# mahbhlddnhakkh/yuv-manipulations-2

Hardware: AMD Instinct MI355X
Metric: megapixels/sec DCT compress+decompress, 4K IYUV; achieved HBM GB/s vs peak (higher is better)
Workload: dtype u8/int16 (fp32 transform)

## Files before the change

### yuv-manipulations-2_amd/csrc/fdct_bfly.h

```cpp
#pragma once

#if defined(__HIPCC__)
#define MYYUV_BF_HD __host__ __device__ __forceinline__
#else
#include <math.h>
#define MYYUV_BF_HD static inline
#endif

#ifndef MYYUV_BFLY_MUTANT
#define MYYUV_BFLY_MUTANT 0
#endif
#if MYYUV_BFLY_MUTANT && defined(__HIPCC__)
#error "MYYUV_BFLY_MUTANT is for the host check only"
#endif
#if MYYUV_BFLY_MUTANT == 1
#define MYYUV_BF_FMA(a, b, c) ((a) * (b) + (c))
#else
#define MYYUV_BF_FMA(a, b, c) fmaf(a, b, c)
#endif

namespace myyuv_bfly {

#if MYYUV_BFLY_MUTANT == 2
constexpr float kC0 = 0.3535533845424652f, kC4 = kC0;
#else
constexpr float kC0 = 0.3535533845424652f, kC4 = 0.3535534143447876f;
#endif
constexpr float kA2 = 0.4619397521018982f, kB2 = 0.19134166836738586f;
constexpr float kA6 = 0.4619397521018982f, kB6 = 0.19134169816970825f;
constexpr float kO1[4] = {0.49039262533187866f, 0.41573476791381836f, 0.27778512239456177f, 0.09754513204097748f};
constexpr float kO3[4] = {0.41573482751846313f, -0.0975450873374939f, -0.49039262533187866f, -0.277785062789917f};
constexpr float kO5[4] = {0.2777852416038513f, -0.49039262533187866f, 0.09754514694213867f, 0.41573476791381836f};
constexpr float kO7[4] = {0.09754543751478195f, -0.2777852416038513f, 0.4157347083091736f, -0.49039262533187866f};
constexpr float kBflyK = 7.946e-7f;

MYYUV_BF_HD float odd4(const float (&o)[4], float d0, float d1, float d2, float d3) {
  return MYYUV_BF_FMA(o[3], d3, MYYUV_BF_FMA(o[2], d2, MYYUV_BF_FMA(o[1], d1, o[0] * d0)));
}

MYYUV_BF_HD void bfly_cols(const float (&p)[8], float (&t)[8]) {
  const float s0 = p[0] + p[7], s1 = p[1] + p[6], s2 = p[2] + p[5], s3 = p[3] + p[4];
  const float d0 = p[0] - p[7], d1 = p[1] - p[6], d2 = p[2] - p[5], d3 = p[3] - p[4];
  const float ss0 = s0 + s3, ss1 = s1 + s2, ds0 = s0 - s3, ds1 = s1 - s2;
  t[0] = kC0 * ((ss0 + ss1) - 1024.0f);
  t[4] = kC4 * (ss0 - ss1);
  t[2] = MYYUV_BF_FMA(kA2, ds0, kB2 * ds1);
  t[6] = MYYUV_BF_FMA(kB6, ds0, -kA6 * ds1);
  t[1] = odd4(kO1, d0, d1, d2, d3);
  t[3] = odd4(kO3, d0, d1, d2, d3);
  t[5] = odd4(kO5, d0, d1, d2, d3);
  t[7] = odd4(kO7, d0, d1, d2, d3);
}

MYYUV_BF_HD void bfly_rows(const float (&x)[8], float (&y)[8]) {
  const float s0 = x[0] + x[7], s1 = x[1] + x[6], s2 = x[2] + x[5], s3 = x[3] + x[4];
  const float d0 = x[0] - x[7], d1 = x[1] - x[6], d2 = x[2] - x[5], d3 = x[3] - x[4];
  const float ss0 = s0 + s3, ss1 = s1 + s2, ds0 = s0 - s3, ds1 = s1 - s2;
  y[0] = kC0 * (ss0 + ss1);
  y[4] = kC4 * (ss0 - ss1);
  y[2] = MYYUV_BF_FMA(kA2, ds0, kB2 * ds1);
  y[6] = MYYUV_BF_FMA(kB6, ds0, -kA6 * ds1);
  y[1] = odd4(kO1, d0, d1, d2, d3);
  y[3] = odd4(kO3, d0, d1, d2, d3);
  y[5] = odd4(kO5, d0, d1, d2, d3);
  y[7] = odd4(kO7, d0, d1, d2, d3);
}

MYYUV_BF_HD void bfly_row_bounds(const float* r, float* kb) {
  for (int i = 0; i < 8; i++) {
    double m = 0.0;
    for (int v = 0; v < 8; v++) m = r[i * 8 + v] > m ? r[i * 8 + v] : m;
    kb[i] = (float)((double)kBflyK * m * (1.0 + 0x1p-20) * (1.0 + 0x1p-22));
  }
}

#if !defined(__HIPCC__)
struct BflyDetail {
  int row, col;
  float dec;
  float a;
  float t[64];
};
static inline int bfly_block(const unsigned char* px, const float* R, const float* kb, short* out,
                             BflyDetail* d = nullptr) {
  unsigned a = 0;
  for (int i = 0; i < 64; i++) a += px[i] > 128 ? px[i] - 128u : 128u - px[i];
  const float af = (float)a;
  float T[8][8];
  for (int k = 0; k < 8; k++) {
    float p[8], t[8];
    for (int m = 0; m < 8; m++) p[m] = (float)px[m * 8 + k];
    bfly_cols(p, t);
    for (int i = 0; i < 8; i++) T[i][k] = t[i];
  }
  int ok = 1;
  for (int i = 0; i < 8; i++) {
    float y[8];
    bfly_rows(T[i], y);
    float em = 0.0f;
    int vm = 0;
    for (int v = 0; v < 8; v++) {
      const float t = y[v] * R[i * 8 + v];
      const float uu = t + 0x1.8p23f;
      const float e = t - (uu - 0x1.8p23f);
      if (fabsf(e) > em) vm = v;
      em = fmaxf(em, fabsf(e));
      out[i * 8 + v] = (short)(int)(uu - 0x1.8p23f);
      if (d) d->t[i * 8 + v] = t;
    }
    const float dec = fmaf(af, kb[i], em);
    if (dec >= 0.5f) ok = 0;
    if (d && (i == 0 || dec > d->dec)) {
      d->row = i;
      d->col = vm;
      d->dec = dec;
    }
  }
  if (d) d->a = af;
  return ok;
}
#endif

}
```

### yuv-manipulations-2_amd/csrc/k1_store.hpp

```cpp
#pragma once
#include "codec_common.hpp"
#include "xform_common.hpp"

namespace myyuv_gpu {
namespace xf {

typedef unsigned short k1_us2 __attribute__((ext_vector_type(2)));

__device__ __forceinline__ void store_block_rows(const uint32_t (&c)[16], uint32_t q, uint32_t lane, bool live,
                                                 uint32_t g, uint4* dlo, uint4* dhi, uint8_t* __restrict__ rmask,
                                                 uint32_t* __restrict__ binfo, const uint4* zq,
                                                 uint4* __restrict__ sink) {
  uint4 lo, hi;
  uint32_t rm;
  pack_quads(c, q, lo, hi, rm);
  const uint4 z0 = zq[0], z1 = zq[1];
  const uint32_t wv[8] = {lo.x, lo.y, lo.z, lo.w, hi.x, hi.y, hi.z, hi.w};
  const uint32_t zv[8] = {z0.x, z0.y, z0.z, z0.w, z1.x, z1.y, z1.z, z1.w};
  k1_us2 cnt = {0, 0}, mx = {0, 0};
#pragma unroll
  for (int i = 0; i < 8; i++) {
    uint32_t fu, m16;
    asm("v_pk_min_u16 %0, %1, %2" : "=v"(fu) : "v"(wv[i]), "s"(0x00010001u));
    cnt += __builtin_bit_cast(k1_us2, fu);
    asm("v_pk_mul_lo_u16 %0, %1, %2" : "=v"(m16) : "v"(fu), "v"(zv[i]));
    mx = __builtin_elementwise_max(mx, __builtin_bit_cast(k1_us2, m16));
  }
  uint32_t nnz = (uint32_t)cnt.x + (uint32_t)cnt.y;
  uint32_t msz = mx.x > mx.y ? (uint32_t)mx.x : (uint32_t)mx.y;
#pragma unroll
  for (int d = 1; d < 4; d <<= 1) {
    const uint32_t o = d == 1 ? quad_xor1(nnz | (msz << 16)) : quad_xor2(nnz | (msz << 16));
    nnz += o & 0xFFFFu;
    msz = max(msz, o >> 16);
  }
  const bool nzl = (rm >> (2 * q)) & 1u, nzh = (rm >> (2 * q + 1)) & 1u;
  *(live ? rmask + g : reinterpret_cast<uint8_t*>(sink + 128) + lane) = (uint8_t)rm;
  const uint32_t dc = quad_lane0(lo.x);
  *(live ? binfo + g : reinterpret_cast<uint32_t*>(sink + 132) + lane) = binfo_word(rm, msz, class_of(nnz, msz), dc);
  *(nzl ? dlo : sink + lane) = lo;
  *(nzh ? dhi : sink + 64 + lane) = hi;
}

#ifndef MYYUV_K1_BUF
#define MYYUV_K1_BUF 1
#endif
typedef unsigned int k1_v4u __attribute__((ext_vector_type(4)));
constexpr uint32_t kOob = 0xFFFFFFFFu;

struct K1Rsrc {
  __amdgpu_buffer_rsrc_t coef, rmask, binfo;
};
__device__ __forceinline__ K1Rsrc k1_rsrc(uint4* coef, uint8_t* rmask, uint32_t* binfo, const FrameGeom& G) {
  const uint32_t nblk = G.cum[3] * G.nframes;
  K1Rsrc r;
  r.coef = __builtin_amdgcn_make_buffer_rsrc(coef, 0, (int)(((nblk + 63u) / 64u) * (kCoefQuadsPerWave * 16u)),
                                             0x00020000);
  r.rmask = __builtin_amdgcn_make_buffer_rsrc(rmask, 0, (int)nblk, 0x00020000);
  r.binfo = __builtin_amdgcn_make_buffer_rsrc(binfo, 0, (int)(nblk * 4u), 0x00020000);
  return r;
}

__device__ __forceinline__ void store_block_rows_buf(const uint32_t (&c)[16], uint32_t q, bool live, uint32_t g,
                                                     const K1Rsrc& R, const uint4* zq) {
  uint4 lo, hi;
  uint32_t rm;
  pack_quads(c, q, lo, hi, rm);
  const uint4 z0 = zq[0], z1 = zq[1];
  const uint32_t wv[8] = {lo.x, lo.y, lo.z, lo.w, hi.x, hi.y, hi.z, hi.w};
  const uint32_t zv[8] = {z0.x, z0.y, z0.z, z0.w, z1.x, z1.y, z1.z, z1.w};
  k1_us2 cnt = {0, 0}, mx = {0, 0};
#pragma unroll
  for (int i = 0; i < 8; i++) {
    uint32_t fu, m16;
    asm("v_pk_min_u16 %0, %1, %2" : "=v"(fu) : "v"(wv[i]), "s"(0x00010001u));
    cnt += __builtin_bit_cast(k1_us2, fu);
    asm("v_pk_mul_lo_u16 %0, %1, %2" : "=v"(m16) : "v"(fu), "v"(zv[i]));
    mx = __builtin_elementwise_max(mx, __builtin_bit_cast(k1_us2, m16));
  }
  uint32_t nnz = (uint32_t)cnt.x + (uint32_t)cnt.y;
  uint32_t msz = mx.x > mx.y ? (uint32_t)mx.x : (uint32_t)mx.y;
#pragma unroll
  for (int d = 1; d < 4; d <<= 1) {
    const uint32_t o = d == 1 ? quad_xor1(nnz | (msz << 16)) : quad_xor2(nnz | (msz << 16));
    nnz += o & 0xFFFFu;
    msz = max(msz, o >> 16);
  }
  const bool nzl = (rm >> (2 * q)) & 1u, nzh = (rm >> (2 * q + 1)) & 1u;
  const uint32_t dc = quad_lane0(lo.x);
  __builtin_amdgcn_raw_buffer_store_b8((uint8_t)rm, R.rmask, live ? g : kOob, 0, 0);
  __builtin_amdgcn_raw_buffer_store_b32(binfo_word(rm, msz, class_of(nnz, msz), dc), R.binfo, live ? 4u * g : kOob,
                                        0, 0);
  const uint32_t qo = coef_quad(g, 2 * q) * 16u;
  __builtin_amdgcn_raw_buffer_store_b128(k1_v4u{lo.x, lo.y, lo.z, lo.w}, R.coef, live && nzl ? qo : kOob, 0, 0);
  __builtin_amdgcn_raw_buffer_store_b128(k1_v4u{hi.x, hi.y, hi.z, hi.w}, R.coef, live && nzh ? qo + 1024u : kOob, 0,
                                         0);
}

__device__ __forceinline__ void stage_zz(uint4* szz) {
  if (threadIdx.x < 32) reinterpret_cast<uint32_t*>(szz)[threadIdx.x] = kZzPairs.v[threadIdx.x];
}

}
}
```

### yuv-manipulations-2_amd/csrc/k_huff_decode.hip

```cpp
#include "codec_common.hpp"
#include "coef_xform.h"
#include "downscale.h"
#include "huff_common.hpp"
#include "idct_scaled.h"
#include "k1_store.hpp"
#include "k_metric.hpp"
#include "k_stream.hpp"
#include "requant.h"
#include "xform_common.hpp"

namespace myyuv_gpu {

namespace {

constexpr uint32_t kStageQuads = 320;
constexpr uint32_t kZeroBit = kStageQuads * 128u;
constexpr uint32_t kGposQuads = 8 * 64 * 4 / 16;

#ifndef MYYUV_K5_GROUP
#define MYYUV_K5_GROUP 2
#endif
#ifndef MYYUV_K5_FORMS
#define MYYUV_K5_FORMS 1
#endif
// ... 1259 lines not shown
        const uint32_t w = v < 2 ? w0 : w1;
        z[u * N + v] = (int16_t)((v & 1) ? w >> 16 : w & 0xFFFFu);
        q[u * N + v] = sqs[8 * u + v];
      }
    }
    uint8_t px[N * N];
    myyuv_scaled::idct_scaled_block<N>(z, q, px);
    if (live) {
#pragma unroll
      for (int i = 0; i < N; i++) {
        uint8_t* o = img + myyuv_downscale::lane_pixel(kDen, r, lane, (uint32_t)i);
        if constexpr (N == 1) {
          o[0] = px[0];
        } else if constexpr (N == 2) {
          *reinterpret_cast<uint16_t*>(o) = (uint16_t)(px[2 * i] | (px[2 * i + 1] << 8));
        } else {
          *reinterpret_cast<uint32_t*>(o) = (uint32_t)px[4 * i] | ((uint32_t)px[4 * i + 1] << 8) |
                                            ((uint32_t)px[4 * i + 2] << 16) | ((uint32_t)px[4 * i + 3] << 24);
        }
      }
    }
  }
  xf::wave_sync();

  const uint32_t q = lane & 3u, b = lane >> 2;
  float* tb = reinterpret_cast<float*>(stq) + b * xf::kTile;
  const xf::K1Rsrc rs = xf::k1_rsrc(coef, rmask, binfo, Gd);
  const uint32_t g0 = blockIdx.y * Gd.cum[3] + (p == 0 ? Gd.cum[0] : (p == 1 ? Gd.cum[1] : Gd.cum[2]));
#pragma unroll 1
  for (uint32_t u0 = 0; u0 < W.nout; u0 += kXfUnit) {
    const uint32_t slot = u0 + b;
    const bool lv = slot < W.nout;
    const uint32_t g = g0 + myyuv_downscale::out_block(W, slot);
    xf::fdct_core(img + 64u * slot, tb, q, sqr, p, [&](const uint32_t (&c)[16], bool keep) {
      xf::store_block_rows_buf(c, q, lv && keep, g, rs, szz + 2 * q);
    });
    xf::wave_sync();
  }
}
#define MYYUV_DOWNSCALE_INST(N)                                                                                   \
  template __global__ void k_downscale<N>(const uint8_t*, const uint32_t*, uint32_t, const StreamDesc*,           \
                                          const uint32_t*, const uint32_t*, FrameGeom, FrameGeom,                 \
                                          myyuv_downscale::Map, const DownscaleTables*, uint4*, uint8_t*,         \
                                          uint32_t*, unsigned long long*);
MYYUV_DOWNSCALE_INST(1)
MYYUV_DOWNSCALE_INST(2)
MYYUV_DOWNSCALE_INST(4)
#undef MYYUV_DOWNSCALE_INST

__global__ __launch_bounds__(64, MYYUV_K5_WAVES) void k_requant(const uint8_t* __restrict__ in,
                                               const uint32_t* __restrict__ in_size,
                                               uint32_t cap,
                                               const StreamDesc* __restrict__ desc,
                                               const uint32_t* __restrict__ local_off,
                                               const uint32_t* __restrict__ tile_pre,
                                               FrameGeom G, uint32_t tiles_p0,
                                               uint32_t tiles_p1, const RequantTables* __restrict__ rt,
                                               uint4* __restrict__ coef,
                                               uint8_t* __restrict__ rmask,
                                               uint32_t* __restrict__ binfo,
                                               unsigned long long* __restrict__ err) {
  __shared__ uint4 stq[kStageQuads + 1 + kGposQuads];
  __shared__ float sqs[64], sqd[64];
  const uint32_t lane = threadIdx.x;
  if (lane == 0) stq[kStageQuads] = make_uint4(0u, 0u, 0u, 0u);
  {
    const uint32_t t = blockIdx.x;
    const int p = t >= tiles_p0 ? (t >= tiles_p0 + tiles_p1 ? 2 : 1) : 0;
// ... 305 lines not shown
```

### yuv-manipulations-2_amd/csrc/k_huff_encode.hip

```cpp
#include "codec_common.hpp"
#ifdef MYYUV_STAMPS
namespace myyuv_gpu {
extern __device__ uint32_t g_k2_fstamps[8192 * 8];
}
#define R8_STAMP_DECL unsigned long long _r8prev = 0;
#define R8_STAMP(k)                                                                   \
  do {                                                                                \
    __builtin_amdgcn_sched_barrier(0);                                                \
    unsigned long long _t = __builtin_amdgcn_s_memtime();                             \
    __builtin_amdgcn_sched_barrier(0);                                                \
    if ((threadIdx.x & 63) == 0 && (k) > 0 && blockIdx.x * (blockDim.x >> 6) + (threadIdx.x >> 6) < 8192) \
      g_k2_fstamps[(blockIdx.x * (blockDim.x >> 6) + (threadIdx.x >> 6)) * 8 + (k)] = (uint32_t)(_t - _r8prev); \
    _r8prev = _t;                                                                     \
  } while (0)
#endif
#include "huff_common.hpp"
#include "huff_r16.hpp"
#include "xform_common.hpp"

namespace myyuv_gpu {

#ifdef MYYUV_STAMPS
__device__ unsigned long long g_k2_stamps[40];
__device__ uint32_t g_k2_fstamps[8192 * 8];
// ... 1127 lines not shown
                                                             const QTables* __restrict__ qt,
                                                             uint4* __restrict__ coef,
                                                             uint8_t* __restrict__ rmask,
                                                             uint32_t* __restrict__ stage,
                                                             uint32_t* __restrict__ tinfo,
                                                             uint8_t* __restrict__ sizes,
                                                             uint32_t* __restrict__ srcoff,
                                                             uint32_t* __restrict__ work,
                                                             uint32_t* __restrict__ work_count) {
  using namespace xf;
  __shared__ uint4 s_img[8 * kK2Group];
  __shared__ float s_tile[kTileWaves][kXfUnit * kTile];
  __shared__ float s_q[kSqWords];
  __shared__ uint8_t s_rmk[kK2Group];
  static_assert(sizeof(TileScratch) <= sizeof(s_tile), "K2 scratch over the transpose tiles");
  const uint32_t tid = threadIdx.x, wave = tid >> 6, lane = tid & 63;
  const uint32_t q = lane & 3u, b = lane >> 2;
  const uint32_t T = blockIdx.y * G.tcum[3] + blockIdx.x;
  uint32_t f, t, g0, nloc;
  int p;
  tile_geometry(G, T, f, t, p, g0, nloc);
  TileRows rows;
  load_tile_rows(frame, G, T, wave, b, q, rows);
  stage_tables<kSqWords>(qt->q[0], s_q);
  float* tb = s_tile[wave] + b * kTile;
  uint8_t* img = reinterpret_cast<uint8_t*>(tb);
#pragma unroll
  for (int i = 0; i < 4; i++) {
    const uint32_t lb = (4 * wave + i) * kXfUnit + b;
    if ((4 * wave + i) * kXfUnit >= nloc) break;
    *reinterpret_cast<uint2*>(img + 16u * q) = make_uint2(rows.px[i].x, rows.px[i].y);
    *reinterpret_cast<uint2*>(img + 16u * q + 8u) = make_uint2(rows.px[i].z, rows.px[i].w);
    wave_sync();
    fdct_core(img, tb, q, s_q, p, [&](const uint32_t (&c)[16], bool) {
      uint4 lo, hi;
      uint32_t rm;
      pack_quads(c, q, lo, hi, rm);
      if (lb < nloc) {
        s_img[(2 * q) * kK2Group + lb] = lo;
        s_img[(2 * q + 1) * kK2Group + lb] = hi;
        if (q == 0) s_rmk[lb] = (uint8_t)rm;
      }
    });
    wave_sync();
  }
  __syncthreads();
  TileScratch& sc = *reinterpret_cast<TileScratch*>(&s_tile[0][0]);
  const LdsCoef src{s_img, s_rmk, coef, rmask, f * G.cum[3] + g0};
  encode_tile(src, sc, T, nloc, stage, tinfo, sizes, srcoff, work, work_count);
}

__global__ __launch_bounds__(kWideLanes) void k_huff_encode_wide(const uint4* __restrict__ coef,
                                                        const uint8_t* __restrict__ rmask,
                                                        const uint4* __restrict__ zq, FrameGeom G,
                                                        uint32_t* __restrict__ oslots,
                                                        uint8_t* __restrict__ sizes,
                                                        uint32_t* __restrict__ tinfo,
                                                        const uint32_t* __restrict__ work,
                                                        const uint32_t* __restrict__ work_count,
                                                        const uint32_t* __restrict__ work2,
                                                        const uint32_t* __restrict__ work2_count,
                                                        uint32_t gate, uint32_t limit) {
  constexpr int CAP = 64;
  __shared__ uint32_t lds[Layout<CAP>::kWords * kWideLanes];
  const OvfList L = overflow_list(work, work_count, work2, work2_count, gate);
  const uint32_t cnt = L.n;
  if (cnt <= limit) return;
  for (uint32_t base = blockIdx.x * kWideLanes; base < cnt; base += gridDim.x * kWideLanes) {
    const uint32_t i = base + threadIdx.x;
    const bool live = i < cnt;
    const uint32_t g = live ? L.ids[i] : 0;
    CoefRegs R;
    R.load(coef, zq, g, live ? rmask[g] : 0u);
// ... 77 lines not shown
```

### yuv-manipulations-2_amd/csrc/k_transform.hip

```cpp
#include <stddef.h>

#include "bmp_fdct.h"
#include "codec_common.hpp"
#include "color_px.hpp"
#include "k1_store.hpp"
#include "k_metric.hpp"
#include "xform_common.hpp"

#ifndef MYYUV_K1_OCC
#define MYYUV_K1_OCC 8
#endif
#define MYYUV_K1_ATTR __attribute__((amdgpu_waves_per_eu(MYYUV_K1_OCC, MYYUV_K1_OCC)))

namespace myyuv_gpu {

using namespace xf;



__global__ __launch_bounds__(256) MYYUV_K1_ATTR void k_fdct_quant(const uint8_t* __restrict__ frame, FrameGeom G,
                                                   const QTables* __restrict__ qt,
                                                   uint4* __restrict__ coef, uint8_t* __restrict__ rmask,
                                                   uint32_t* __restrict__ binfo, uint4* __restrict__ sink,
                                                   uint32_t* __restrict__ k2ctl, uint32_t* __restrict__ fix,
// ... 2 lines not shown
  __shared__ float tile[4][kXfUnit * kTile];
  __shared__ float sqr[kSqWords];
  __shared__ uint4 szz[8];
  static_assert(offsetof(QTables, r) == sizeof(float) * kSqR && offsetof(QTables, kb) == sizeof(float) * kSqKb,
                "layout");
  stage_zz(szz);
  stage_tables<kSqWords>(qt->q[0], sqr);
  if (kSinkSlots > 1) sink += (size_t)((blockIdx.x * 4u + (threadIdx.x >> 6)) % kSinkSlots) * kSinkQuads;
  const uint32_t lane = threadIdx.x & 63u;
  const uint32_t q = lane & 3u, b = lane >> 2;
  float* tb = tile[threadIdx.x >> 6] + b * kTile;
  uint8_t* img = reinterpret_cast<uint8_t*>(tb);
#if MYYUV_K1_BUF
  const K1Rsrc rs = k1_rsrc(coef, rmask, binfo, G);
#endif
  const uint32_t nall = G.ucum[3] * G.nframes, stride = unit_stride();
  uint32_t ua = first_unit();
  uint4 nx = ua < nall ? load_rows(frame, G, ua, b, q) : make_uint4(0, 0, 0, 0);
  sink[lane] = make_uint4(0, 0, 0, 0);
  sink[64 + lane] = make_uint4(0, 0, 0, 0);
  reinterpret_cast<uint8_t*>(sink + 128)[lane] = 0;

  for (; ua < nall; ua += stride) {
    const uint32_t f = div_magic(ua, G.umag);
    const Unit U = unit_of(G, ua - f * G.ucum[3]);
    const uint32_t local = U.local0 + b;
    const bool live = local < U.nb;
    const uint32_t g = f * G.cum[3] + U.cum + local;
    *reinterpret_cast<uint2*>(img + 16u * q) = make_uint2(nx.x, nx.y);
    *reinterpret_cast<uint2*>(img + 16u * q + 8u) = make_uint2(nx.z, nx.w);
    nx = load_rows(frame, G, ua + stride < nall ? ua + stride : ua, b, q);
    wave_sync();

    auto store = [&](const uint32_t (&c)[16], bool keep) {
      const bool lv = live && keep;
#if MYYUV_K1_BUF
      store_block_rows_buf(c, q, lv, g, rs, szz + 2 * q);
#else
      uint4* dlo = lv ? coef + coef_quad(g, 2 * q) : sink + lane;
      uint4* dhi = lv ? coef + coef_quad(g, 2 * q + 1) : sink + 64 + lane;
      store_block_rows(c, q, lane, lv, g, dlo, dhi, rmask, binfo, szz + 2 * q, sink);
#endif
    };
    uint32_t xr[4];
    fdct_load(img, q, xr);
    const uint64_t bad = fdct_fast<true>(xr, tb, q, sqr, U.p, store);
    if (bad != 0) {
      const bool mine = ((bad >> lane) & 1u) && q == 0 && live;
      const uint64_t m = __ballot(mine);
      const uint32_t c = ua % kFixLists;
      uint32_t base = 0;
      if (lane == 0 && m != 0) base = atomicAdd(fix_count(fix, par, c), (uint32_t)__popcll(m));
      base = __builtin_amdgcn_readfirstlane(base);
      const uint32_t idx = base + __builtin_amdgcn_mbcnt_hi((uint32_t)(m >> 32), __builtin_amdgcn_mbcnt_lo((uint32_t)m, 0u));
      if (mine && idx < fix_list_cap(nall)) fix_list(fix, G, c)[idx] = ua * kXfUnit + b;
    }
  }
}

__global__ __launch_bounds__(64 * kFixWaves) void k_fdct_fix(const uint8_t* __restrict__ frame, FrameGeom G,
                                                  const QTables* __restrict__ qt, uint4* __restrict__ coef,
                                                  uint8_t* __restrict__ rmask, uint32_t* __restrict__ binfo,
                                                  uint4* __restrict__ sink,
                                                  uint32_t* __restrict__ fix, uint32_t par) {
  __shared__ float tile[kFixWaves][kXfUnit * kTile];
  __shared__ float sqr[2 * 3 * 64];
  __shared__ uint4 szz[8];
  __shared__ uint32_t s_any;
  if (blockIdx.x == 0 && threadIdx.x < kFixLists) *fix_count(fix, par ^ 1u, threadIdx.x) = 0u;
  if (threadIdx.x == 0) s_any = 0u;
  __syncthreads();
  const uint32_t gw = blockIdx.x * kFixWaves + (threadIdx.x >> 6), nw = gridDim.x * kFixWaves;
  const uint32_t c = gw % kFixLists;
  const uint32_t n = __builtin_amdgcn_readfirstlane(*fix_count(fix, par, c));
  if ((threadIdx.x & 63u) == 0 && gw / kFixLists * kXfUnit < n) s_any = 1u;
  __syncthreads();
  if (s_any == 0u) return;
  stage_zz(szz);
#pragma unroll
  for (uint32_t i = threadIdx.x; i < 2u * 3u * 64u; i += 64u * kFixWaves) sqr[i] = qt->q[0][i];
  __syncthreads();
  const uint32_t lane = threadIdx.x & 63u;
  const uint32_t q = lane & 3u, b = lane >> 2;
  float* tb = tile[threadIdx.x >> 6] + b * kTile;
  uint8_t* img = reinterpret_cast<uint8_t*>(tb);
  const uint32_t* list = fix_list(fix, G, c);
#if MYYUV_K1_BUF
  const K1Rsrc rs = k1_rsrc(coef, rmask, binfo, G);
#endif
  for (uint32_t i = gw / kFixLists * kXfUnit; i < n; i += nw / kFixLists * kXfUnit) {
    const bool real = i + b < n;
    const uint32_t ent = list[real ? i + b : i];
    const uint32_t ua = ent / kXfUnit, bb = ent % kXfUnit;
    const uint32_t f = div_magic(ua, G.umag);
    const Unit U = unit_of(G, ua - f * G.ucum[3]);
    const uint32_t g = f * G.cum[3] + U.cum + U.local0 + bb;
    const uint4 r = load_rows(frame, G, ua, bb, q);
    wave_sync();
    *reinterpret_cast<uint2*>(img + 16u * q) = make_uint2(r.x, r.y);
    *reinterpret_cast<uint2*>(img + 16u * q + 8u) = make_uint2(r.z, r.w);
    wave_sync();
    uint32_t xr[4];
    fdct_load(img, q, xr);
#if MYYUV_K1_BUF
    fdct_exact(xr, tb, q, sqr, U.p, [&](const uint32_t (&cc)[16]) { store_block_rows_buf(cc, q, real, g, rs, szz + 2 * q); });
#else
    uint4* dlo = real ? coef + coef_quad(g, 2 * q) : sink + lane;
    uint4* dhi = real ? coef + coef_quad(g, 2 * q + 1) : sink + 64 + lane;
    fdct_exact(xr, tb, q, sqr, U.p,
               [&](const uint32_t (&cc)[16]) {
                 store_block_rows(cc, q, lane, real, g, dlo, dhi, rmask, binfo, szz + 2 * q, sink);
               });
#endif
  }
}

template <class Out>
__device__ __forceinline__ void dequant_idct_units(const uint4* __restrict__ coef,
                                                   const uint8_t* __restrict__ rmask,
                                                   const uint4* __restrict__ zq, const FrameGeom& G,
                                                   float (*tile)[kXfUnit * kTile], const float* sq,
                                                   uint4* __restrict__ sink, Out& out) {
  const uint32_t lane = threadIdx.x & 63u;
  const uint32_t q = lane & 3u, b = lane >> 2;
  float* tb = tile[threadIdx.x >> 6] + b * kTile;
  uint32_t* tw = reinterpret_cast<uint32_t*>(tb);
  const uint32_t nall = G.ucum[3] * G.nframes, stride = unit_stride();
  uint32_t ua = first_unit();
  uint4 na = make_uint4(0, 0, 0, 0), nc = na;
  uint32_t un = ua + stride < nall ? ua + stride : ua, nm = 0;
  if (ua < nall) {
    const uint32_t g0 = unit_block(G, ua, b);
    load_quads(coef, zq, g0, q, rmask[g0], na, nc);
    nm = rmask[unit_block(G, un, b)];
  }
  sink[lane] = make_uint4(0, 0, 0, 0);
  sink[64 + lane] = make_uint4(0, 0, 0, 0);

  for (; ua < nall; ua += stride) {
    const uint32_t f = div_magic(ua, G.umag);
    const Unit U = unit_of(G, ua - f * G.ucum[3]);
    const uint32_t local = U.local0 + b;
    *reinterpret_cast<uint4*>(tw + 8 * q) = na;
    *reinterpret_cast<uint4*>(tw + 8 * q + 4) = nc;
// ... 184 lines not shown
    for (uint32_t t0 = 0; t0 < bf::kTileRows; t0 += kDepth) {
      uint32_t w[kDepth][2][BPP];
#pragma unroll
      for (uint32_t i = 0; i < kDepth; i++)
#pragma unroll
        for (uint32_t dr = 0; dr < 2; dr++) px::load4<BPP>(fr + (int64_t)(2 * (t0 + i) + dr) * step, 0, w[i][dr]);
#pragma unroll
      for (uint32_t i = 0; i < kDepth; i++) {
        const uint32_t ty = t0 + i;
        uint32_t Y[2] = {0, 0}, cb[2] = {0, 0}, cr[2] = {0, 0};
        px::tile_row<BPP>(w[i][0], M.orient == 1, Y[0], cb, cr);
        px::tile_row<BPP>(w[i][1], M.orient == 1, Y[1], cb, cr);
        *reinterpret_cast<uint32_t*>(img + bf::luma_byte(S, lane, ty, 0)) = Y[0];
        *reinterpret_cast<uint32_t*>(img + bf::luma_byte(S, lane, ty, 1)) = Y[1];
        uint8_t* uc = img + bf::chroma_byte(lane, ty);
        *reinterpret_cast<uint16_t*>(uc) = (uint16_t)((cb[0] & 0xFFu) | (cb[1] & 0xFFu) << 8);
        *reinterpret_cast<uint16_t*>(uc + (bf::kSlotV - bf::kSlotU) * bf::kSlotBytes) =
            (uint16_t)((cr[0] & 0xFFu) | (cr[1] & 0xFFu) << 8);
      }
    }
  }
  wave_sync();

  const uint32_t q = lane & 3u, b = lane >> 2;
  float* tb = tile + b * kTile;
  const K1Rsrc rs = k1_rsrc(coef, rmask, binfo, G);
  const uint32_t nu = bf::units(S);
#pragma unroll 1
  for (uint32_t k = 0; k < nu; k++) {
    const bf::UnitOf U = bf::unit_of(S, k);
    const bool lv = b < U.nlive;
    const uint32_t g = blockIdx.y * G.cum[3] + (U.p == 0 ? G.cum[0] : (U.p == 1 ? G.cum[1] : G.cum[2])) +
                       bf::plane_block(M, S, U, lv ? b : 0u);
    fdct_core(img + bf::kSlotBytes * (U.slot0 + b), tb, q, sqr, U.p, [&](const uint32_t (&c)[16], bool keep) {
      store_block_rows_buf(c, q, lv && keep, g, rs, szz + 2 * q);
    });
    wave_sync();
  }
}

template __global__ void k_bmp_fdct<3>(const uint8_t*, myyuv_bmpfdct::Map, FrameGeom, const QTables*, uint4*, uint8_t*,
                                       uint32_t*);
template __global__ void k_bmp_fdct<4>(const uint8_t*, myyuv_bmpfdct::Map, FrameGeom, const QTables*, uint4*, uint8_t*,
                                       uint32_t*);

}
```

### yuv-manipulations-2_amd/csrc/xform_common.hpp

```cpp
#pragma once
#include <stddef.h>

#include "codec_common.hpp"
#include "fdct_bfly.h"

namespace myyuv_gpu {
namespace xf {

constexpr float c_dct[64] = MYYUV_DCT_MATRIX;
constexpr int kTile = 72;
constexpr int kXfTile16 = 16 * kTile;
constexpr float kMagic = 0x1.8p23f;
constexpr float kMagicPx = 0x1.8p23f + 128.0f;
constexpr float kHalfDown = 0x1.fffffep-2f;

__device__ __forceinline__ constexpr int tix(int i, int j) { return (i >> 1) * 18 + 2 * j + (i & 1); }

__device__ __forceinline__ uint32_t bits(float x) { return __builtin_bit_cast(uint32_t, x); }

__device__ __forceinline__ void wave_sync() {
  __builtin_amdgcn_fence(__ATOMIC_RELEASE, "wavefront");
  __builtin_amdgcn_wave_barrier();
  __builtin_amdgcn_fence(__ATOMIC_ACQUIRE, "wavefront");
}
// ... 67 lines not shown
  }
#pragma unroll
  for (int k = 0; k < 8; k++) {
    if (kSkip && (kFence || k >= kAlwaysSteps) && !__any(P[2 * k] != 0.0f || P[2 * k + 1] != 0.0f)) continue;
    float pr[16];
#pragma unroll
    for (int v = 0; v < 8; v++) {
      const float d = c_dct[kInverse ? k * 8 + v : v * 8 + k];
      pr[2 * v] = P[2 * k] * d;
      pr[2 * v + 1] = P[2 * k + 1] * d;
    }
#pragma unroll
    for (int j = 0; j < 16; j++) out[j] = (k == 0 && !kSkip) ? pr[j] : out[j] + pr[j];
    if (kFence) fence16(out);
  }
}

__device__ __forceinline__ void transpose_tile(float* tb, uint32_t q, const float (&M)[16],
                                               float (&P)[16]) {
#pragma unroll
  for (int i = 0; i < 8; i++) {
    tb[tix(i, 2 * q)] = M[2 * i];
    tb[tix(i, 2 * q + 1)] = M[2 * i + 1];
  }
  wave_sync();
#pragma unroll
  for (int k = 0; k < 8; k++) {
    const float2 v = *reinterpret_cast<const float2*>(tb + tix(2 * q, k));
    P[2 * k] = v.x;
    P[2 * k + 1] = v.y;
  }
}

__device__ __forceinline__ float sbyte(uint32_t w, int k) {
  return (float)(int)(int8_t)(uint8_t)(w >> (8 * k));
}

__device__ __forceinline__ uint4 load_rows(const uint8_t* __restrict__ frame, const FrameGeom& G,
                                           uint32_t ua, uint32_t b, uint32_t q) {
  const uint32_t f = div_magic(ua, G.umag);
  const Unit U = unit_of(G, ua - f * G.ucum[3]);
  const uint32_t local = U.local0 + b;
  const uint32_t off = block_row_offset(U, local < U.nb ? local : U.nb - 1, 2u * q);
  const uint8_t* fr = frame + (size_t)f * G.fbytes;
  const uint2 r0 = *reinterpret_cast<const uint2*>(fr + off);
  const uint2 r1 = *reinterpret_cast<const uint2*>(fr + off + U.pw);
  return make_uint4(r0.x, r0.y, r1.x, r1.y);
}

template <int kWords>
__device__ __forceinline__ void stage_tables(const float* __restrict__ src, float* dst) {
  static_assert(kWords <= 512, "two words per thread of the 256-thread workgroup");
#pragma unroll
  for (uint32_t i = threadIdx.x; i < 512u; i += 256u)
    if (i < (uint32_t)kWords) dst[i] = src[i];
  __syncthreads();
}

__device__ __forceinline__ uint32_t unit_block(const FrameGeom& G, uint32_t ua, uint32_t b) {
  const uint32_t f = div_magic(ua, G.umag);
  const Unit U = unit_of(G, ua - f * G.ucum[3]);
  const uint32_t local = U.local0 + b;
  return f * G.cum[3] + U.cum + (local < U.nb ? local : U.nb - 1);
}

__device__ __forceinline__ void load_quads(const uint4* __restrict__ coef, const uint4* __restrict__ zq,
                                           uint32_t g, uint32_t q, uint32_t m, uint4& a, uint4& c) {
  const uint4* pa = (m >> (2 * q)) & 1u ? coef + coef_quad(g, 2 * q) : zq;
  const uint4* pc = (m >> (2 * q + 1)) & 1u ? coef + coef_quad(g, 2 * q + 1) : zq;
  a = *pa;
  c = *pc;
}


__device__ __forceinline__ void fdct_stage1_exact(const uint32_t (&xr)[4], float (&T)[16]) {
#pragma unroll
  for (int k = 0; k < 8; k++) {
    const uint32_t w = xr[k >> 1] ^ 0x80808080u;
    const float x0 = sbyte(w, 2 * (k & 1)), x1 = sbyte(w, 2 * (k & 1) + 1);
#pragma unroll
    for (int i = 0; i < 8; i++) {
      const float d = c_dct[i * 8 + k];
      const float p0 = d * x0, p1 = d * x1;
      T[2 * i] = k == 0 ? p0 : T[2 * i] + p0;
      T[2 * i + 1] = k == 0 ? p1 : T[2 * i + 1] + p1;
    }
    fence16(T);
  }
}


__device__ __forceinline__ void fdct_load(const uint8_t* img, uint32_t q, uint32_t (&xr)[4]) {
#pragma unroll
  for (int m = 0; m < 4; m++)
    xr[m] = *reinterpret_cast<const uint16_t*>(img + 16 * m + 2 * q) |
            ((uint32_t)*reinterpret_cast<const uint16_t*>(img + 16 * m + 8 + 2 * q) << 16);
  wave_sync();
}

constexpr int kSqR = 3 * 64, kSqKb = 2 * 3 * 64, kSqWords = 2 * 3 * 64 + 3 * 8;

template <bool kPerBlock, class Emit>
__device__ __forceinline__ uint64_t fdct_fast(const uint32_t (&xr)[4], float* tb, uint32_t q, const float* sqr, int p,
                                              Emit&& emit) {
  uint32_t a = 0;
#pragma unroll
  for (int m = 0; m < 4; m++) a = __builtin_amdgcn_sad_u8(xr[m], 0x80808080u, a);
  a += quad_xor1(a);
  a += quad_xor2(a);
  float T[16];
#pragma unroll
  for (int c = 0; c < 2; c++) {
    float px[8], t[8];
#pragma unroll
    for (int m = 0; m < 8; m++) px[m] = (float)((xr[m >> 1] >> (8 * (2 * (m & 1) + c))) & 0xFFu);
    myyuv_bfly::bfly_cols(px, t);
#pragma unroll
    for (int i = 0; i < 8; i++) T[2 * i + c] = t[i];
  }
  float P[16];
  transpose_tile(tb, q, T, P);
  const float af = (float)a;
  const float* Rq = sqr + kSqR + p * 64 + 16u * q;
  uint32_t c[16];
  float mx = 0.0f;
#pragma unroll
  for (int h = 0; h < 2; h++) {
    float x[8], y[8];
#pragma unroll
    for (int k = 0; k < 8; k++) x[k] = P[2 * k + h];
    myyuv_bfly::bfly_rows(x, y);
    float em = 0.0f;
#pragma unroll
    for (int v = 0; v < 8; v++) {
      const float t = y[v] * Rq[8 * h + v];
      const float u = t + kMagic;
      const float e = t - (u - kMagic);
      em = __builtin_fmaxf(em, __builtin_fabsf(e));
      c[2 * v + h] = bits(u);
    }
    mx = __builtin_fmaxf(mx, __builtin_fmaf(af, sqr[kSqKb + p * 8 + 2 * q + h], em));
  }
  const uint64_t bad = __builtin_amdgcn_ballot_w64(mx >= 0.5f);
  if (bad == 0) {
    emit(c, true);
    return 0;
  }
  if (!kPerBlock) return bad;
  uint32_t fb = mx >= 0.5f ? 1u : 0u;
  fb |= quad_xor1(fb);
  fb |= quad_xor2(fb);
  emit(c, fb == 0u);
  return __builtin_amdgcn_ballot_w64(fb != 0u);
}

template <class Emit>
__device__ __forceinline__ void fdct_exact(const uint32_t (&xr)[4], float* tb, uint32_t q, const float* sqr, int p,
                                           Emit&& emit) {
  const uint32_t n0 = 16u * q;
  float T[16];
  fdct_stage1_exact(xr, T);
  float P[16];
  transpose_tile(tb, q, T, P);
  float Y[16];
  dot_rows<false>(P, Y);
  const float4* R4 = reinterpret_cast<const float4*>(sqr + kSqR + p * 64 + n0);
  const float4 r0 = R4[0], r1 = R4[1], r2 = R4[2], r3 = R4[3];
  const float rr[16] = {r0.x, r2.x, r0.y, r2.y, r0.z, r2.z, r0.w, r2.w,
                        r1.x, r3.x, r1.y, r3.y, r1.z, r3.z, r1.w, r3.w};
  uint32_t c[16];
  float mx = 0.0f;
#pragma unroll
  for (int j = 0; j < 16; j++) {
    const float tq = Y[j] * rr[j];
    const float uu = tq + kMagic;
    const float e = tq - (uu - kMagic);
    mx = __builtin_fmaxf(mx, __builtin_fmaf(__builtin_fabsf(tq), kNearRel, __builtin_fabsf(e)));
    c[j] = bits(uu);
  }
  if (mx >= 0.5f) {
    const float* Qt = sqr + p * 64 + n0;
#pragma unroll
    for (int j = 0; j < 16; j++) c[j] = (uint32_t)(int)roundf(Y[j] / Qt[(j >> 1) + 8 * (j & 1)]);
  }
  emit(c);
}

template <class Emit>
__device__ __forceinline__ void fdct_core(const uint8_t* img, float* tb, uint32_t q, const float* sqr, int p,
                                          Emit&& emit) {
  uint32_t xr[4];
  fdct_load(img, q, xr);
  if (__builtin_expect(fdct_fast<false>(xr, tb, q, sqr, p, emit) != 0, 0)) {
    wave_sync();
    fdct_exact(xr, tb, q, sqr, p, [&](const uint32_t (&c)[16]) { emit(c, true); });
  }
}

__device__ __forceinline__ void pack_quads(const uint32_t (&c)[16], uint32_t q, uint4& lo, uint4& hi,
                                           uint32_t& rm) {
  lo.x = __builtin_amdgcn_perm(c[2], c[0], 0x05040100u);
  lo.y = __builtin_amdgcn_perm(c[6], c[4], 0x05040100u);
  lo.z = __builtin_amdgcn_perm(c[10], c[8], 0x05040100u);
  lo.w = __builtin_amdgcn_perm(c[14], c[12], 0x05040100u);
  hi.x = __builtin_amdgcn_perm(c[3], c[1], 0x05040100u);
  hi.y = __builtin_amdgcn_perm(c[7], c[5], 0x05040100u);
  hi.z = __builtin_amdgcn_perm(c[11], c[9], 0x05040100u);
  hi.w = __builtin_amdgcn_perm(c[15], c[13], 0x05040100u);
  const bool nzl = (lo.x | lo.y | lo.z | lo.w) != 0u, nzh = (hi.x | hi.y | hi.z | hi.w) != 0u;
  rm = (nzl ? 1u << (2 * q) : 0u) | (nzh ? 2u << (2 * q) : 0u);
  rm |= quad_xor1(rm);
  rm |= quad_xor2(rm);
}

__device__ __forceinline__ constexpr uint32_t img_word(uint32_t b) { return 4u * ((b >> 2) & 1u); }

__device__ __forceinline__ void idct_rows(float* tb, uint32_t q, uint32_t b, const float* Qt, uint2& w0,
                                          uint2& w1) {
  const uint32_t* tw = reinterpret_cast<const uint32_t*>(tb) + img_word(b);
  uint32_t zc[8];
#pragma unroll
  for (int k = 0; k < 8; k++) zc[k] = tw[k * 4 + q];
  wave_sync();
  float qk[16];
#pragma unroll
  for (int k = 0; k < 8; k++) {
    const float2 v = *reinterpret_cast<const float2*>(Qt + k * 8 + 2 * q);
    qk[2 * k] = v.x;
    qk[2 * k + 1] = v.y;
  }

  float Um[16];
#pragma unroll
  for (int j = 0; j < 16; j++) Um[j] = 0.0f;
#pragma unroll
  for (int k = 0; k < 8; k++) {
    if (k >= kAlwaysSteps && !__any(zc[k] != 0u)) continue;
    const float z0 = (float)(int16_t)zc[k] * qk[2 * k];
    const float z1 = (float)(int16_t)(zc[k] >> 16) * qk[2 * k + 1];
    float pr[16];
#pragma unroll
    for (int i = 0; i < 8; i++) {
      pr[2 * i] = c_dct[k * 8 + i] * z0;
// ... 97 lines not shown
```

Before: 392,900.

## Skip high-half DCT rows proven zero and remap row-to-lane layout

The forward DCT now assigns rows q and q+4 to each lane instead of rows 2q and 2q+1, using a new transpose. A bound test on the column-pass output proves whether rows 4-7 quantize to zero for the whole wave. If so, it skips the second row butterfly, packing, counting and the high coefficient store. Coefficient quad indexing, the row mask bits and the zigzag table indexing change to match across the transform, encode and decode kernels. The gate only fires for coarse quantizers, and the extra ballot and bound check add cost when it does not fire.

```diff
diff --git a/yuv-manipulations-2_amd/csrc/fdct_bfly.h b/yuv-manipulations-2_amd/csrc/fdct_bfly.h
--- a/yuv-manipulations-2_amd/csrc/fdct_bfly.h
+++ b/yuv-manipulations-2_amd/csrc/fdct_bfly.h
@@ -33,6 +33,11 @@
 constexpr float kO5[4] = {0.2777852416038513f, -0.49039262533187866f, 0.09754514694213867f, 0.41573476791381836f};
 constexpr float kO7[4] = {0.09754543751478195f, -0.2777852416038513f, 0.4157347083091736f, -0.49039262533187866f};
 constexpr float kBflyK = 7.946e-7f;
+#if MYYUV_BFLY_MUTANT == 3
+constexpr float kZeroRowK = 0.5f * 617157.8125f;
+#else
+constexpr float kZeroRowK = 617157.8125f;
+#endif
 
 MYYUV_BF_HD float odd4(const float (&o)[4], float d0, float d1, float d2, float d3) {
   return MYYUV_BF_FMA(o[3], d3, MYYUV_BF_FMA(o[2], d2, MYYUV_BF_FMA(o[1], d1, o[0] * d0)));
@@ -73,6 +78,16 @@
     kb[i] = (float)((double)kBflyK * m * (1.0 + 0x1p-20) * (1.0 + 0x1p-22));
   }
 }
+
+MYYUV_BF_HD float bfly_zero_row_dec(const float (&x)[8], float a, float kb) {
+  const float s = ((fabsf(x[0]) + fabsf(x[1])) + (fabsf(x[2]) + fabsf(x[3]))) +
+                  ((fabsf(x[4]) + fabsf(x[5])) + (fabsf(x[6]) + fabsf(x[7])));
+  return kb * fmaf(s, kZeroRowK, a);
+}
+MYYUV_BF_HD bool bfly_zero_row(const float (&x)[8], float a, float kb) { return bfly_zero_row_dec(x, a, kb) < 0.5f; }
+
+constexpr float kZeroRowGate = kBflyK / 5.5f;
+MYYUV_BF_HD bool bfly_zero_rows_tested(float kb4) { return kb4 < kZeroRowGate; }
 
 #if !defined(__HIPCC__)
 struct BflyDetail {
@@ -119,6 +134,23 @@
   if (d) d->a = af;
   return ok;
 }
+static inline int bfly_block_zero_rows(const unsigned char* px, const float* kb, float* dec = nullptr) {
+  unsigned a = 0;
+  for (int i = 0; i < 64; i++) a += px[i] > 128 ? px[i] - 128u : 128u - px[i];
+  float T[8][8];
+  for (int k = 0; k < 8; k++) {
+    float p[8], t[8];
+    for (int m = 0; m < 8; m++) p[m] = (float)px[m * 8 + k];
+    bfly_cols(p, t);
+    for (int i = 0; i < 8; i++) T[i][k] = t[i];
+  }
+  int votes = 0;
+  for (int i = 4; i < 8; i++) {
+    if (dec) dec[i - 4] = bfly_zero_row_dec(T[i], (float)a, kb[i]);
+    if (bfly_zero_row(T[i], (float)a, kb[i])) votes |= 1 << (i - 4);
+  }
+  return votes;
+}
 #endif
 
 }
diff --git a/yuv-manipulations-2_amd/csrc/k1_store.hpp b/yuv-manipulations-2_amd/csrc/k1_store.hpp
--- a/yuv-manipulations-2_amd/csrc/k1_store.hpp
+++ b/yuv-manipulations-2_amd/csrc/k1_store.hpp
@@ -7,19 +7,20 @@
 
 typedef unsigned short k1_us2 __attribute__((ext_vector_type(2)));
 
+template <bool kHiZero = false>
 __device__ __forceinline__ void store_block_rows(const uint32_t (&c)[16], uint32_t q, uint32_t lane, bool live,
                                                  uint32_t g, uint4* dlo, uint4* dhi, uint8_t* __restrict__ rmask,
-                                                 uint32_t* __restrict__ binfo, const uint4* zq,
+                                                 uint32_t* __restrict__ binfo, const uint4* szz,
                                                  uint4* __restrict__ sink) {
   uint4 lo, hi;
   uint32_t rm;
-  pack_quads(c, q, lo, hi, rm);
-  const uint4 z0 = zq[0], z1 = zq[1];
+  pack_quads<kHiZero>(c, q, lo, hi, rm);
+  const uint4 z0 = szz[q], z1 = szz[kHiZero ? q : q + 4];
   const uint32_t wv[8] = {lo.x, lo.y, lo.z, lo.w, hi.x, hi.y, hi.z, hi.w};
   const uint32_t zv[8] = {z0.x, z0.y, z0.z, z0.w, z1.x, z1.y, z1.z, z1.w};
   k1_us2 cnt = {0, 0}, mx = {0, 0};
 #pragma unroll
-  for (int i = 0; i < 8; i++) {
+  for (int i = 0; i < (kHiZero ? 4 : 8); i++) {
     uint32_t fu, m16;
     asm("v_pk_min_u16 %0, %1, %2" : "=v"(fu) : "v"(wv[i]), "s"(0x00010001u));
     cnt += __builtin_bit_cast(k1_us2, fu);
@@ -34,12 +35,12 @@
     nnz += o & 0xFFFFu;
     msz = max(msz, o >> 16);
   }
-  const bool nzl = (rm >> (2 * q)) & 1u, nzh = (rm >> (2 * q + 1)) & 1u;
+  const bool nzl = (rm >> q) & 1u, nzh = (rm >> (q + 4)) & 1u;
   *(live ? rmask + g : reinterpret_cast<uint8_t*>(sink + 128) + lane) = (uint8_t)rm;
   const uint32_t dc = quad_lane0(lo.x);
   *(live ? binfo + g : reinterpret_cast<uint32_t*>(sink + 132) + lane) = binfo_word(rm, msz, class_of(nnz, msz), dc);
   *(nzl ? dlo : sink + lane) = lo;
-  *(nzh ? dhi : sink + 64 + lane) = hi;
+  if (!kHiZero) *(nzh ? dhi : sink + 64 + lane) = hi;
 }
 
 #ifndef MYYUV_K1_BUF
@@ -61,17 +62,18 @@
   return r;
 }
 
+template <bool kHiZero = false>
 __device__ __forceinline__ void store_block_rows_buf(const uint32_t (&c)[16], uint32_t q, bool live, uint32_t g,
-                                                     const K1Rsrc& R, const uint4* zq) {
+                                                     const K1Rsrc& R, const uint4* szz) {
   uint4 lo, hi;
   uint32_t rm;
-  pack_quads(c, q, lo, hi, rm);
-  const uint4 z0 = zq[0], z1 = zq[1];
+  pack_quads<kHiZero>(c, q, lo, hi, rm);
+  const uint4 z0 = szz[q], z1 = szz[kHiZero ? q : q + 4];
   const uint32_t wv[8] = {lo.x, lo.y, lo.z, lo.w, hi.x, hi.y, hi.z, hi.w};
   const uint32_t zv[8] = {z0.x, z0.y, z0.z, z0.w, z1.x, z1.y, z1.z, z1.w};
   k1_us2 cnt = {0, 0}, mx = {0, 0};
 #pragma unroll
-  for (int i = 0; i < 8; i++) {
+  for (int i = 0; i < (kHiZero ? 4 : 8); i++) {
     uint32_t fu, m16;
     asm("v_pk_min_u16 %0, %1, %2" : "=v"(fu) : "v"(wv[i]), "s"(0x00010001u));
     cnt += __builtin_bit_cast(k1_us2, fu);
@@ -86,15 +88,16 @@
     nnz += o & 0xFFFFu;
     msz = max(msz, o >> 16);
   }
-  const bool nzl = (rm >> (2 * q)) & 1u, nzh = (rm >> (2 * q + 1)) & 1u;
+  const bool nzl = (rm >> q) & 1u, nzh = (rm >> (q + 4)) & 1u;
   const uint32_t dc = quad_lane0(lo.x);
   __builtin_amdgcn_raw_buffer_store_b8((uint8_t)rm, R.rmask, live ? g : kOob, 0, 0);
   __builtin_amdgcn_raw_buffer_store_b32(binfo_word(rm, msz, class_of(nnz, msz), dc), R.binfo, live ? 4u * g : kOob,
                                         0, 0);
-  const uint32_t qo = coef_quad(g, 2 * q) * 16u;
+  const uint32_t qo = coef_quad(g, q) * 16u;
   __builtin_amdgcn_raw_buffer_store_b128(k1_v4u{lo.x, lo.y, lo.z, lo.w}, R.coef, live && nzl ? qo : kOob, 0, 0);
-  __builtin_amdgcn_raw_buffer_store_b128(k1_v4u{hi.x, hi.y, hi.z, hi.w}, R.coef, live && nzh ? qo + 1024u : kOob, 0,
-                                         0);
+  if (!kHiZero)
+    __builtin_amdgcn_raw_buffer_store_b128(k1_v4u{hi.x, hi.y, hi.z, hi.w}, R.coef, live && nzh ? qo + 4096u : kOob, 0,
+                                           0);
 }
 
 __device__ __forceinline__ void stage_zz(uint4* szz) {
diff --git a/yuv-manipulations-2_amd/csrc/k_huff_decode.hip b/yuv-manipulations-2_amd/csrc/k_huff_decode.hip
--- a/yuv-manipulations-2_amd/csrc/k_huff_decode.hip
+++ b/yuv-manipulations-2_amd/csrc/k_huff_decode.hip
@@ -1315,8 +1315,8 @@
     const uint32_t slot = u0 + b;
     const bool lv = slot < W.nout;
     const uint32_t g = g0 + myyuv_downscale::out_block(W, slot);
-    xf::fdct_core(img + 64u * slot, tb, q, sqr, p, [&](const uint32_t (&c)[16], bool keep) {
-      xf::store_block_rows_buf(c, q, lv && keep, g, rs, szz + 2 * q);
+    xf::fdct_core(img + 64u * slot, tb, q, lv, sqr, p, [&](const uint32_t (&c)[16], bool keep, auto hz) {
+      xf::store_block_rows_buf<decltype(hz)::value>(c, q, lv && keep, g, rs, szz);
     });
     xf::wave_sync();
   }
diff --git a/yuv-manipulations-2_amd/csrc/k_huff_encode.hip b/yuv-manipulations-2_amd/csrc/k_huff_encode.hip
--- a/yuv-manipulations-2_amd/csrc/k_huff_encode.hip
+++ b/yuv-manipulations-2_amd/csrc/k_huff_encode.hip
@@ -1183,13 +1183,13 @@
     *reinterpret_cast<uint2*>(img + 16u * q) = make_uint2(rows.px[i].x, rows.px[i].y);
     *reinterpret_cast<uint2*>(img + 16u * q + 8u) = make_uint2(rows.px[i].z, rows.px[i].w);
     wave_sync();
-    fdct_core(img, tb, q, s_q, p, [&](const uint32_t (&c)[16], bool) {
+    fdct_core(img, tb, q, lb < nloc, s_q, p, [&](const uint32_t (&c)[16], bool, auto hz) {
       uint4 lo, hi;
       uint32_t rm;
-      pack_quads(c, q, lo, hi, rm);
+      pack_quads<decltype(hz)::value>(c, q, lo, hi, rm);
       if (lb < nloc) {
-        s_img[(2 * q) * kK2Group + lb] = lo;
-        s_img[(2 * q + 1) * kK2Group + lb] = hi;
+        s_img[q * kK2Group + lb] = lo;
+        s_img[(q + 4) * kK2Group + lb] = hi;
         if (q == 0) s_rmk[lb] = (uint8_t)rm;
       }
     });
diff --git a/yuv-manipulations-2_amd/csrc/k_transform.hip b/yuv-manipulations-2_amd/csrc/k_transform.hip
--- a/yuv-manipulations-2_amd/csrc/k_transform.hip
+++ b/yuv-manipulations-2_amd/csrc/k_transform.hip
@@ -58,19 +58,20 @@
     nx = load_rows(frame, G, ua + stride < nall ? ua + stride : ua, b, q);
     wave_sync();
 
-    auto store = [&](const uint32_t (&c)[16], bool keep) {
+    auto store = [&](const uint32_t (&c)[16], bool keep, auto hz) {
+      constexpr bool kHz = decltype(hz)::value;
       const bool lv = live && keep;
 #if MYYUV_K1_BUF
-      store_block_rows_buf(c, q, lv, g, rs, szz + 2 * q);
+      store_block_rows_buf<kHz>(c, q, lv, g, rs, szz);
 #else
-      uint4* dlo = lv ? coef + coef_quad(g, 2 * q) : sink + lane;
-      uint4* dhi = lv ? coef + coef_quad(g, 2 * q + 1) : sink + 64 + lane;
-      store_block_rows(c, q, lane, lv, g, dlo, dhi, rmask, binfo, szz + 2 * q, sink);
+      uint4* dlo = lv ? coef + coef_quad(g, q) : sink + lane;
+      uint4* dhi = lv ? coef + coef_quad(g, q + 4) : sink + 64 + lane;
+      store_block_rows<kHz>(c, q, lane, lv, g, dlo, dhi, rmask, binfo, szz, sink);
 #endif
     };
     uint32_t xr[4];
     fdct_load(img, q, xr);
-    const uint64_t bad = fdct_fast<true>(xr, tb, q, sqr, U.p, store);
+    const uint64_t bad = fdct_fast<true>(xr, tb, q, live, sqr, U.p, store);
     if (bad != 0) {
       const bool mine = ((bad >> lane) & 1u) && q == 0 && live;
       const uint64_t m = __ballot(mine);
@@ -129,13 +130,13 @@
     uint32_t xr[4];
     fdct_load(img, q, xr);
 #if MYYUV_K1_BUF
-    fdct_exact(xr, tb, q, sqr, U.p, [&](const uint32_t (&cc)[16]) { store_block_rows_buf(cc, q, real, g, rs, szz + 2 * q); });
+    fdct_exact(xr, tb, q, sqr, U.p, [&](const uint32_t (&cc)[16]) { store_block_rows_buf(cc, q, real, g, rs, szz); });
 #else
-    uint4* dlo = real ? coef + coef_quad(g, 2 * q) : sink + lane;
-    uint4* dhi = real ? coef + coef_quad(g, 2 * q + 1) : sink + 64 + lane;
+    uint4* dlo = real ? coef + coef_quad(g, q) : sink + lane;
+    uint4* dhi = real ? coef + coef_quad(g, q + 4) : sink + 64 + lane;
     fdct_exact(xr, tb, q, sqr, U.p,
                [&](const uint32_t (&cc)[16]) {
-                 store_block_rows(cc, q, lane, real, g, dlo, dhi, rmask, binfo, szz + 2 * q, sink);
+                 store_block_rows(cc, q, lane, real, g, dlo, dhi, rmask, binfo, szz, sink);
                });
 #endif
   }
@@ -386,9 +387,10 @@
     const bool lv = b < U.nlive;
     const uint32_t g = blockIdx.y * G.cum[3] + (U.p == 0 ? G.cum[0] : (U.p == 1 ? G.cum[1] : G.cum[2])) +
                        bf::plane_block(M, S, U, lv ? b : 0u);
-    fdct_core(img + bf::kSlotBytes * (U.slot0 + b), tb, q, sqr, U.p, [&](const uint32_t (&c)[16], bool keep) {
-      store_block_rows_buf(c, q, lv && keep, g, rs, szz + 2 * q);
-    });
+    fdct_core(img + bf::kSlotBytes * (U.slot0 + b), tb, q, lv, sqr, U.p,
+              [&](const uint32_t (&c)[16], bool keep, auto hz) {
+                store_block_rows_buf<decltype(hz)::value>(c, q, lv && keep, g, rs, szz);
+              });
     wave_sync();
   }
 }
diff --git a/yuv-manipulations-2_amd/csrc/xform_common.hpp b/yuv-manipulations-2_amd/csrc/xform_common.hpp
--- a/yuv-manipulations-2_amd/csrc/xform_common.hpp
+++ b/yuv-manipulations-2_amd/csrc/xform_common.hpp
@@ -123,6 +123,23 @@
   }
 }
 
+__device__ __forceinline__ constexpr int tixf(int i, int j) { return (i & 3) * 18 + 2 * j + (i >> 2); }
+
+__device__ __forceinline__ void transpose_fwd(float* tb, uint32_t q, const float (&M)[16], float (&P)[16]) {
+#pragma unroll
+  for (int i = 0; i < 8; i++) {
+    tb[tixf(i, 2 * q)] = M[2 * i];
+    tb[tixf(i, 2 * q + 1)] = M[2 * i + 1];
+  }
+  wave_sync();
+#pragma unroll
+  for (int k = 0; k < 8; k++) {
+    const float2 v = *reinterpret_cast<const float2*>(tb + tixf(q, k));
+    P[2 * k] = v.x;
+    P[2 * k + 1] = v.y;
+  }
+}
+
 __device__ __forceinline__ float sbyte(uint32_t w, int k) {
   return (float)(int)(int8_t)(uint8_t)(w >> (8 * k));
 }
@@ -180,6 +197,10 @@
   }
 }
 
+template <bool kZero>
+struct HiZero {
+  static constexpr bool value = kZero;
+};
 
 __device__ __forceinline__ void fdct_load(const uint8_t* img, uint32_t q, uint32_t (&xr)[4]) {
 #pragma unroll
@@ -192,8 +213,8 @@
 constexpr int kSqR = 3 * 64, kSqKb = 2 * 3 * 64, kSqWords = 2 * 3 * 64 + 3 * 8;
 
 template <bool kPerBlock, class Emit>
-__device__ __forceinline__ uint64_t fdct_fast(const uint32_t (&xr)[4], float* tb, uint32_t q, const float* sqr, int p,
-                                              Emit&& emit) {
+__device__ __forceinline__ uint64_t fdct_fast(const uint32_t (&xr)[4], float* tb, uint32_t q, bool live,
+                                              const float* sqr, int p, Emit&& emit) {
   uint32_t a = 0;
 #pragma unroll
   for (int m = 0; m < 4; m++) a = __builtin_amdgcn_sad_u8(xr[m], 0x80808080u, a);
@@ -210,13 +231,13 @@
     for (int i = 0; i < 8; i++) T[2 * i + c] = t[i];
   }
   float P[16];
-  transpose_tile(tb, q, T, P);
+  transpose_fwd(tb, q, T, P);
   const float af = (float)a;
-  const float* Rq = sqr + kSqR + p * 64 + 16u * q;
+  const float* Rq = sqr + kSqR + p * 64 + 8u * q;
+  const float* kb = sqr + kSqKb + p * 8 + q;
   uint32_t c[16];
-  float mx = 0.0f;
-#pragma unroll
-  for (int h = 0; h < 2; h++) {
+  auto row = [&](auto hc) {
+    constexpr int h = decltype(hc)::value ? 1 : 0;
     float x[8], y[8];
 #pragma unroll
     for (int k = 0; k < 8; k++) x[k] = P[2 * k + h];
@@ -224,39 +245,57 @@
     float em = 0.0f;
 #pragma unroll
     for (int v = 0; v < 8; v++) {
-      const float t = y[v] * Rq[8 * h + v];
+      const float t = y[v] * Rq[32 * h + v];
       const float u = t + kMagic;
       const float e = t - (u - kMagic);
       em = __builtin_fmaxf(em, __builtin_fabsf(e));
       c[2 * v + h] = bits(u);
     }
-    mx = __builtin_fmaxf(mx, __builtin_fmaf(af, sqr[kSqKb + p * 8 + 2 * q + h], em));
-  }
-  const uint64_t bad = __builtin_amdgcn_ballot_w64(mx >= 0.5f);
-  if (bad == 0) {
-    emit(c, true);
-    return 0;
-  }
-  if (!kPerBlock) return bad;
-  uint32_t fb = mx >= 0.5f ? 1u : 0u;
-  fb |= quad_xor1(fb);
-  fb |= quad_xor2(fb);
-  emit(c, fb == 0u);
-  return __builtin_amdgcn_ballot_w64(fb != 0u);
+    return __builtin_fmaf(af, kb[4 * h], em);
+  };
+  auto finish = [&](float mx, auto hz) -> uint64_t {
+    const uint64_t bad = __builtin_amdgcn_ballot_w64(mx >= 0.5f);
+    if (bad == 0) {
+      emit(c, true, hz);
+      return 0;
+    }
+    if (!kPerBlock) return bad;
+    uint32_t fb = mx >= 0.5f ? 1u : 0u;
+    fb |= quad_xor1(fb);
+    fb |= quad_xor2(fb);
+    emit(c, fb == 0u, hz);
+    return __builtin_amdgcn_ballot_w64(fb != 0u);
+  };
+  bool skip = false;
+  const float kb4 = __builtin_bit_cast(float, __builtin_amdgcn_readfirstlane(bits(sqr[kSqKb + p * 8 + 4])));
+  if (myyuv_bfly::bfly_zero_rows_tested(kb4)) {
+    float x1[8];
+#pragma unroll
+    for (int k = 0; k < 8; k++) x1[k] = P[2 * k + 1];
+    const bool zr = myyuv_bfly::bfly_zero_row(x1, af, kb[4]) || !live;
+    skip = __builtin_amdgcn_ballot_w64(zr) == ~0ull;
+  }
+  const float m0 = row(HiZero<false>{});
+  if (skip) {
+#pragma unroll
+    for (int v = 0; v < 8; v++) c[2 * v + 1] = 0u;
+    return finish(m0, HiZero<true>{});
+  }
+  return finish(__builtin_fmaxf(m0, row(HiZero<true>{})), HiZero<false>{});
 }
 
 template <class Emit>
 __device__ __forceinline__ void fdct_exact(const uint32_t (&xr)[4], float* tb, uint32_t q, const float* sqr, int p,
                                            Emit&& emit) {
-  const uint32_t n0 = 16u * q;
+  const uint32_t n0 = 8u * q;
   float T[16];
   fdct_stage1_exact(xr, T);
   float P[16];
-  transpose_tile(tb, q, T, P);
+  transpose_fwd(tb, q, T, P);
   float Y[16];
   dot_rows<false>(P, Y);
   const float4* R4 = reinterpret_cast<const float4*>(sqr + kSqR + p * 64 + n0);
-  const float4 r0 = R4[0], r1 = R4[1], r2 = R4[2], r3 = R4[3];
+  const float4 r0 = R4[0], r1 = R4[1], r2 = R4[8], r3 = R4[9];
   const float rr[16] = {r0.x, r2.x, r0.y, r2.y, r0.z, r2.z, r0.w, r2.w,
                         r1.x, r3.x, r1.y, r3.y, r1.z, r3.z, r1.w, r3.w};
   uint32_t c[16];
@@ -272,34 +311,38 @@
   if (mx >= 0.5f) {
     const float* Qt = sqr + p * 64 + n0;
 #pragma unroll
-    for (int j = 0; j < 16; j++) c[j] = (uint32_t)(int)roundf(Y[j] / Qt[(j >> 1) + 8 * (j & 1)]);
+    for (int j = 0; j < 16; j++) c[j] = (uint32_t)(int)roundf(Y[j] / Qt[(j >> 1) + 32 * (j & 1)]);
   }
   emit(c);
 }
 
 template <class Emit>
-__device__ __forceinline__ void fdct_core(const uint8_t* img, float* tb, uint32_t q, const float* sqr, int p,
-                                          Emit&& emit) {
+__device__ __forceinline__ void fdct_core(const uint8_t* img, float* tb, uint32_t q, bool live, const float* sqr,
+                                          int p, Emit&& emit) {
   uint32_t xr[4];
   fdct_load(img, q, xr);
-  if (__builtin_expect(fdct_fast<false>(xr, tb, q, sqr, p, emit) != 0, 0)) {
+  if (__builtin_expect(fdct_fast<false>(xr, tb, q, live, sqr, p, emit) != 0, 0)) {
     wave_sync();
-    fdct_exact(xr, tb, q, sqr, p, [&](const uint32_t (&c)[16]) { emit(c, true); });
-  }
-}
-
+    fdct_exact(xr, tb, q, sqr, p, [&](const uint32_t (&c)[16]) { emit(c, true, HiZero<false>{}); });
+  }
+}
+
+template <bool kHiZero = false>
 __device__ __forceinline__ void pack_quads(const uint32_t (&c)[16], uint32_t q, uint4& lo, uint4& hi,
                                            uint32_t& rm) {
   lo.x = __builtin_amdgcn_perm(c[2], c[0], 0x05040100u);
   lo.y = __builtin_amdgcn_perm(c[6], c[4], 0x05040100u);
   lo.z = __builtin_amdgcn_perm(c[10], c[8], 0x05040100u);
   lo.w = __builtin_amdgcn_perm(c[14], c[12], 0x05040100u);
-  hi.x = __builtin_amdgcn_perm(c[3], c[1], 0x05040100u);
-  hi.y = __builtin_amdgcn_perm(c[7], c[5], 0x05040100u);
-  hi.z = __builtin_amdgcn_perm(c[11], c[9], 0x05040100u);
-  hi.w = __builtin_amdgcn_perm(c[15], c[13], 0x05040100u);
-  const bool nzl = (lo.x | lo.y | lo.z | lo.w) != 0u, nzh = (hi.x | hi.y | hi.z | hi.w) != 0u;
-  rm = (nzl ? 1u << (2 * q) : 0u) | (nzh ? 2u << (2 * q) : 0u);
+  hi = make_uint4(0, 0, 0, 0);
+  if (!kHiZero) {
+    hi.x = __builtin_amdgcn_perm(c[3], c[1], 0x05040100u);
+    hi.y = __builtin_amdgcn_perm(c[7], c[5], 0x05040100u);
+    hi.z = __builtin_amdgcn_perm(c[11], c[9], 0x05040100u);
+    hi.w = __builtin_amdgcn_perm(c[15], c[13], 0x05040100u);
+  }
+  const bool nzl = (lo.x | lo.y | lo.z | lo.w) != 0u, nzh = !kHiZero && (hi.x | hi.y | hi.z | hi.w) != 0u;
+  rm = (nzl ? 1u << q : 0u) | (nzh ? 16u << q : 0u);
   rm |= quad_xor1(rm);
   rm |= quad_xor2(rm);
 }
```

Result: faster. 400,500, median of 6 (+2.0%).
